# shahcompbio/MultiModalMuSig.jl

Hardware: AMD Instinct MI355X
Metric: E-step docs/sec (higher is better)
Workload: dtype f64; 1 GPU; LDA K=10 alpha=eta=0.1, 10000 docs x 96 SNV terms (BASELINE configs[1]), nnz(rank 0)=913480, one EM iteration per step; docs_rank0=10000, docs_total=10000, terms=96, topics=10, allreduce=none, comm_nranks=1, devices_visible=1

## Files before the change

include/mmmusig.h:

```cpp
#ifndef MMMUSIG_H
#define MMMUSIG_H

#include <stddef.h>
#include <stdint.h>

#ifdef __cplusplus
extern "C" {
#endif

#define MMM_VERSION 123

enum {
    MMM_OK = 0,
    MMM_DEFERRED = 1,
    MMM_ERR_ARG = -1,
    MMM_ERR_HIP = -2,
    MMM_ERR_RCCL = -3,
    MMM_ERR_UNSUPPORTED = -4,
    MMM_ERR_NUMERIC = -5,
    MMM_ERR_NO_DEVICE = -6
};

typedef struct mmm_ctx mmm_ctx;
typedef struct mmm_lda mmm_lda;
typedef struct mmm_ctm mmm_ctm;

int mmm_version(void);
int mmm_ctx_create(int device_id, mmm_ctx** out);
int mmm_ctx_destroy(mmm_ctx* ctx);
const char* mmm_last_error(const mmm_ctx* ctx);
int mmm_ctx_synchronize(mmm_ctx* ctx);
void* mmm_ctx_stream(mmm_ctx* ctx);
int mmm_ctx_device_name(mmm_ctx* ctx, char* buf, size_t n);

enum { MMM_BUILD_AUTO = 0,
       MMM_BUILD_SPARSE = 1,
       MMM_BUILD_DENSE = 2,
       MMM_BUILD_WIDE = 3 };
enum {
    MMM_OFF_LDA_PADDED_ROWS = 1 << 0,
    MMM_OFF_LDA_COUNT_ROWS = 1 << 1,
    MMM_OFF_LDA_ROWS16 = 1 << 2,
    MMM_OFF_LDA_LL_JOIN = 1 << 3,
    MMM_OFF_LDA_MERGED = 1 << 4,
    MMM_OFF_P2P_FOLDED = 1 << 5,
    MMM_OFF_CTM_PACKED = 1 << 6,
    MMM_OFF_CTM_CPL = 1 << 7,
    MMM_OFF_CTM_KFIT = 1 << 8,
    MMM_OFF_CTM_FUSED_GAUSS = 1 << 9,
    MMM_OFF_CTM_LL_ROWS = 1 << 10,
    MMM_OFF_LDA_EARLY_PROLOGUE = 1 << 11,
    MMM_OFF_CTM_PIPE_GAUSS = 1 << 12,
    MMM_OFF_CTM_SOLVE_ORDER = 1 << 13,
    MMM_OFF_ALL = (1 << 14) - 1
};
typedef struct {
    int lda_build;
    int ctm_build;
    int geometry_cus;
    int grid_blocks;
    int waves_per_block;
    int moment_blocks;
    int side_stream;
    int resident_cap;
    unsigned disable;
    int solve_lanes;
    int solve_waves;
    int reserved[5];
} mmm_tuning_opts;
void mmm_tuning_opts_default(mmm_tuning_opts* o);
int mmm_ctx_set_tuning(mmm_ctx* ctx, const mmm_tuning_opts* opts);
int mmm_ctx_get_tuning(const mmm_ctx* ctx, mmm_tuning_opts* out);
int mmm_ctx_profile_begin(mmm_ctx* ctx);
int mmm_ctx_profile_repeat(mmm_ctx* ctx, int repeat);
int mmm_ctx_profile_select(mmm_ctx* ctx, int phase);
int mmm_ctx_profile_end_phases(mmm_ctx* ctx, int n_spans[8], double total_ms[8]);
int mmm_ctx_profile_end(mmm_ctx* ctx, int* n_launches, double* total_ms);

#define MMM_UNIQUE_ID_BYTES 128
int mmm_comm_unique_id(char out[MMM_UNIQUE_ID_BYTES]);
int mmm_comm_init_rank(mmm_ctx* ctx, int nranks, int rank, const char id[MMM_UNIQUE_ID_BYTES]);
int mmm_comm_nranks(const mmm_ctx* ctx);
#define MMM_P2P_HANDLE_BYTES 64
const char* mmm_comm_transport(const mmm_ctx* ctx);
int mmm_p2p_local_handle(mmm_ctx* ctx, int nranks, char out[MMM_P2P_HANDLE_BYTES]);
int mmm_p2p_attach(mmm_ctx* ctx, int nranks, int rank, const char* handles);
int mmm_p2p_selftest(mmm_ctx* ctx, int* ok);
// ... 2 lines not shown
enum {
    MMM_LDA_LAMBDA = 0,
    MMM_LDA_ELNBETA = 1,
    MMM_LDA_BETA = 2,
    MMM_LDA_GAMMA = 3,
    MMM_LDA_ELNTHETA = 4,
    MMM_LDA_THETA = 5,
    MMM_LDA_PHI = 6,
    MMM_ILDA_LAMBDA = 7, MMM_ILDA_ELNBETA = 8, MMM_ILDA_BETA = 9
};
int mmm_lda_create(mmm_ctx* ctx, int D, int V, int K, double alpha, double eta, const int64_t* doc_ptr,
                   const int32_t* term, const int32_t* count, const double* lambda0, mmm_lda** out);
int mmm_ilda_create(mmm_ctx* ctx, int D, int V, int K, double alpha, int I, const int* J, const double* eta,
                    const int32_t* features, const int64_t* doc_ptr, const int32_t* term, const int32_t* count,
                    const double* lambda0, mmm_lda** out);
int mmm_lda_destroy(mmm_lda* m);
int mmm_lda_get(mmm_lda* m, int field, double* host, size_t n);
int mmm_lda_set(mmm_lda* m, int field, const double* host, size_t n);
int mmm_lda_set_hyper(mmm_lda* m, double alpha, const double* eta, int n_eta);
int mmm_lda_update_gamma(mmm_lda* m);
int mmm_lda_update_phi(mmm_lda* m);
int mmm_lda_update_lambda(mmm_lda* m);
int mmm_lda_update_beta(mmm_lda* m);
int mmm_lda_update_Elntheta(mmm_lda* m);
int mmm_lda_update_Elnbeta(mmm_lda* m);
int mmm_lda_update_theta(mmm_lda* m);
int mmm_lda_loglik(mmm_lda* m, double* ll);
int mmm_lda_elbo(mmm_lda* m, double* elbo, double terms[7]);
int mmm_lda_iterate(mmm_lda* m, int n_iter);
int mmm_lda_ll_history(mmm_lda* m, double* ll, int max_n, int* n);
int mmm_lda_geometry(const mmm_lda* m, int out[8]);
int mmm_lda_row_bytes(const mmm_lda* m);
int mmm_lda_prologue_moved(const mmm_lda* m);
int mmm_lda_fit(mmm_lda* m, int maxiter, double tol, double* ll_hist, int* n_iter, int* converged,
                double* elbo);
int mmm_lda_infer(mmm_lda* m, int unsmoothed, int maxiter, double tol, double* ll_hist, int* n_iter,
                  int* converged);

int mmm_lda_create_batch(mmm_ctx* ctx, int R, int D, int V, int K, double alpha, double eta, const int64_t* doc_ptr,
                         const int32_t* term, const int32_t* count, const double* lambda0, mmm_lda** out);
int mmm_lda_replicas(const mmm_lda* m);
int mmm_lda_select(mmm_lda* m, int r);
int mmm_lda_fit_batch(mmm_lda* m, int maxiter, double tol, double* ll_hist, int* n_iter, int* converged, double* elbo);

typedef struct {
    double xtol_rel;
    double xtol_abs;
    double nu_lower;
    int xtol_rule;
    int max_eval;
} mmm_solver_opts;
void mmm_solver_opts_default(mmm_solver_opts* o);

enum {
    MMM_CTM_MU = 0, MMM_CTM_SIGMA = 1, MMM_CTM_INVSIGMA = 2, MMM_CTM_GAMMA = 3, MMM_CTM_ELNPHI = 4,
    MMM_CTM_PHI = 5, MMM_CTM_LAMBDA = 6, MMM_CTM_NU = 7, MMM_CTM_ZETA = 8, MMM_CTM_PROPS = 9,
    MMM_CTM_THETA = 10, MMM_CTM_ALPHA = 11
};
int mmm_ctm_create(mmm_ctx* ctx, int D, int M, const int* K, const int* V, const double* alpha,
                   const int64_t* doc_ptr, const int32_t* term, const int32_t* count, const int* n_feat,
                   const int* J, const int32_t* features, const double* gamma0, const mmm_solver_opts* opts,
                   mmm_ctm** out);
int mmm_ctm_destroy(mmm_ctm* m);
int mmm_ctm_get(mmm_ctm* m, int field, double* host, size_t n);
int mmm_ctm_set(mmm_ctm* m, int field, const double* host, size_t n);
int mmm_ctm_update_zeta(mmm_ctm* m);
// ... 76 lines not shown
```

multimodalmusig.jl_amd/_lib.py:

```python
import ctypes as C
import os
import subprocess

import numpy as np

_HERE = os.path.dirname(os.path.abspath(__file__))
LIB_PATH = os.environ.get("MMM_LIB_PATH") or os.path.join(_HERE, "lib", "libmmmusig_hip.so")
_LIB = None

f64p = np.ctypeslib.ndpointer(dtype=np.float64, flags="C_CONTIGUOUS")
i64p = np.ctypeslib.ndpointer(dtype=np.int64, flags="C_CONTIGUOUS")
i32p = np.ctypeslib.ndpointer(dtype=np.int32, flags="C_CONTIGUOUS")
vp = C.c_void_p


class MmmError(RuntimeError):
    pass


class SolverOpts(C.Structure):
    _fields_ = [("xtol_rel", C.c_double), ("xtol_abs", C.c_double), ("nu_lower", C.c_double),
                ("xtol_rule", C.c_int), ("max_eval", C.c_int)]


# ... 15 lines not shown
    "mmm_ctx_stream": (vp, [vp]),
    "mmm_ctx_device_name": (C.c_int, [vp, C.c_char_p, C.c_size_t]),
    "mmm_ctx_profile_begin": (C.c_int, [vp]),
    "mmm_ctx_profile_repeat": (C.c_int, [vp, C.c_int]),
    "mmm_ctx_profile_select": (C.c_int, [vp, C.c_int]),
    "mmm_ctx_profile_end_phases": (C.c_int, [vp, C.POINTER(C.c_int), C.POINTER(C.c_double)]),
    "mmm_ctx_profile_end": (C.c_int, [vp, C.POINTER(C.c_int), C.POINTER(C.c_double)]),
    "mmm_comm_unique_id": (C.c_int, [C.c_char_p]),
    "mmm_comm_init_rank": (C.c_int, [vp, C.c_int, C.c_int, C.c_char_p]),
    "mmm_comm_transport": (C.c_char_p, [vp]),
    "mmm_p2p_local_handle": (C.c_int, [vp, C.c_int, C.c_char_p]),
    "mmm_p2p_attach": (C.c_int, [vp, C.c_int, C.c_int, C.c_char_p]),
    "mmm_p2p_selftest": (C.c_int, [vp, C.POINTER(C.c_int)]),
    "mmm_p2p_enable": (C.c_int, [vp, C.c_int]),
    "mmm_comm_nranks": (C.c_int, [vp]),
    "mmm_lda_create": (C.c_int, [vp, C.c_int, C.c_int, C.c_int, C.c_double, C.c_double, i64p, vp, vp, f64p, C.POINTER(vp)]),
    "mmm_ilda_create": (C.c_int, [vp, C.c_int, C.c_int, C.c_int, C.c_double, C.c_int, i32p, f64p, i32p, i64p, vp, vp, f64p, C.POINTER(vp)]),
    "mmm_lda_destroy": (C.c_int, [vp]),
    "mmm_lda_get": (C.c_int, [vp, C.c_int, f64p, C.c_size_t]),
    "mmm_lda_set": (C.c_int, [vp, C.c_int, f64p, C.c_size_t]),
    "mmm_lda_set_hyper": (C.c_int, [vp, C.c_double, f64p, C.c_int]),
    "mmm_lda_update_gamma": (C.c_int, [vp]),
    "mmm_lda_update_phi": (C.c_int, [vp]),
    "mmm_lda_update_lambda": (C.c_int, [vp]),
    "mmm_lda_update_beta": (C.c_int, [vp]),
    "mmm_lda_update_theta": (C.c_int, [vp]),
    "mmm_lda_loglik": (C.c_int, [vp, C.POINTER(C.c_double)]),
    "mmm_lda_elbo": (C.c_int, [vp, C.POINTER(C.c_double), vp]),
    "mmm_lda_iterate": (C.c_int, [vp, C.c_int]),
    "mmm_lda_ll_history": (C.c_int, [vp, vp, C.c_int, C.POINTER(C.c_int)]),
    "mmm_lda_geometry": (C.c_int, [vp, C.POINTER(C.c_int)]),
    "mmm_lda_row_bytes": (C.c_int, [vp]),
    "mmm_lda_prologue_moved": (C.c_int, [vp]),
    "mmm_lda_fit": (C.c_int, [vp, C.c_int, C.c_double, vp, C.POINTER(C.c_int), C.POINTER(C.c_int), C.POINTER(C.c_double)]),
    "mmm_solver_opts_default": (None, [C.POINTER(SolverOpts)]),
    "mmm_lda_infer": (C.c_int, [vp, C.c_int, C.c_int, C.c_double, vp, C.POINTER(C.c_int), C.POINTER(C.c_int)]),
    "mmm_ctm_create": (C.c_int, [vp, C.c_int, C.c_int, i32p, i32p, f64p, i64p, vp, vp, vp, vp, vp, f64p, C.POINTER(SolverOpts), C.POINTER(vp)]),
    "mmm_ctm_destroy": (C.c_int, [vp]),
    "mmm_ctm_get": (C.c_int, [vp, C.c_int, f64p, C.c_size_t]),
    "mmm_ctm_set": (C.c_int, [vp, C.c_int, f64p, C.c_size_t]),
    "mmm_ctm_update_zeta": (C.c_int, [vp]),
    "mmm_ctm_update_theta": (C.c_int, [vp]),
    "mmm_ctm_update_nu": (C.c_int, [vp]),
    "mmm_ctm_update_lambda": (C.c_int, [vp]),
    "mmm_ctm_update_mu": (C.c_int, [vp]),
    "mmm_ctm_update_Sigma": (C.c_int, [vp]),
    "mmm_ctm_update_gamma": (C.c_int, [vp]),
    "mmm_ctm_update_Elnphi": (C.c_int, [vp]),
    "mmm_ctm_update_props": (C.c_int, [vp]),
    "mmm_ctm_update_alpha": (C.c_int, [vp]),
    "mmm_ctm_update_phi": (C.c_int, [vp]),
    "mmm_ctm_loglik": (C.c_int, [vp, f64p]),
    "mmm_ctm_elbo": (C.c_int, [vp, C.POINTER(C.c_double), vp]),
    "mmm_ctm_objectives": (C.c_int, [vp, C.c_int, C.POINTER(C.c_double), f64p, C.POINTER(C.c_double), f64p]),
    "mmm_ctm_geometry": (C.c_int, [vp, C.POINTER(C.c_int)]),
    "mmm_debug_math": (C.c_int, [vp, C.c_int, C.c_size_t, f64p, vp, f64p]),
    "mmm_ctm_solver_stats": (C.c_int, [vp, C.POINTER(C.c_int64), C.POINTER(C.c_int64), C.POINTER(C.c_int64), vp, vp]),
    "mmm_ctm_events": (C.c_int, [vp, C.POINTER(C.c_int64)]),
    "mmm_lda_events": (C.c_int, [vp, C.POINTER(C.c_int64)]),
    "mmm_ctm_iterate": (C.c_int, [vp, C.c_int, C.c_int]),
    "mmm_ctm_ll_history": (C.c_int, [vp, vp, C.c_int, C.POINTER(C.c_int)]),
    "mmm_ctm_fit": (C.c_int, [vp, C.c_int, C.c_double, C.c_int, vp, C.POINTER(C.c_int), C.POINTER(C.c_int), C.POINTER(C.c_double)]),
    "mmm_ctm_infer": (C.c_int, [vp, C.c_int, C.c_int, C.c_double, vp, C.POINTER(C.c_int), C.POINTER(C.c_int)]),
    "mmm_ctm_create_batch": (C.c_int, [vp, C.c_int, C.c_int, C.c_int, i32p, i32p, f64p, i64p, vp, vp, vp, vp, vp, f64p, C.POINTER(SolverOpts), C.POINTER(vp)]),
    "mmm_ctm_replicas": (C.c_int, [vp]),
    "mmm_ctm_select": (C.c_int, [vp, C.c_int]),
# ... 35 lines not shown

def lib():
    global _LIB
    if _LIB is not None:
        return _LIB
    if not os.path.exists(LIB_PATH):
        raise MmmError("libmmmusig_hip.so is not built (%s missing): run `python -c 'import __graft_entry__ as g; g.build()'` "
                       "or `make -C multimodalmusig.jl_amd/csrc`. There is no CPU fallback." % LIB_PATH)
    L = C.CDLL(LIB_PATH, mode=C.RTLD_GLOBAL)
    for name, (res, args) in _SIGS.items():
        fn = getattr(L, name)
        fn.restype = res
        fn.argtypes = args
    _LIB = L
    return L


def check(rc, ctx_handle=None, what=""):
    if rc != 0:
        msg = lib().mmm_last_error(ctx_handle)
        raise MmmError("%s failed with status %d: %s" % (what or "libmmmusig_hip call", rc, (msg or b"").decode(errors="replace")))


_ALL_CTX = []


class TuningOpts(C.Structure):
    _fields_ = [("lda_build", C.c_int), ("ctm_build", C.c_int), ("geometry_cus", C.c_int), ("grid_blocks", C.c_int), ("waves_per_block", C.c_int),
                ("moment_blocks", C.c_int), ("side_stream", C.c_int), ("resident_cap", C.c_int), ("disable", C.c_uint), ("solve_lanes", C.c_int), ("solve_waves", C.c_int), ("reserved", C.c_int * 5)]


BUILDS = {"auto": 0, "sparse": 1, "dense": 2, "wide": 3}
OFF = {"lda_padded_rows": 1 << 0, "lda_count_rows": 1 << 1, "lda_rows16": 1 << 2, "lda_ll_join": 1 << 3, "lda_merged": 1 << 4, "p2p_folded": 1 << 5,
       "ctm_packed": 1 << 6, "ctm_cpl": 1 << 7, "ctm_kfit": 1 << 8, "ctm_fused_gauss": 1 << 9, "ctm_ll_rows": 1 << 10, "lda_early_prologue": 1 << 11, "ctm_pipe_gauss": 1 << 12, "ctm_solve_order": 1 << 13}


class Context:

    def __init__(self, device=0):
        self.h = vp()
        rc = lib().mmm_ctx_create(int(device), C.byref(self.h))
        if rc != 0:
            msg = lib().mmm_last_error(None)
            raise MmmError("mmm_ctx_create(device=%d) failed with status %d: %s -- the HIP path is the only path; "
                           "no CPU fallback exists" % (device, rc, (msg or b"").decode(errors="replace")))
        self.device = int(device)
        self.nranks, self.rank = 1, 0
        _ALL_CTX.append(self)

    def synchronize(self):
        check(lib().mmm_ctx_synchronize(self.h), self.h, "mmm_ctx_synchronize")

    def set_tuning(self, lda_build="auto", ctm_build="auto", geometry_cus=0, grid_blocks=0, waves_per_block=0, moment_blocks=0, side_stream=0,
                   resident_cap=0, disable=(), solve_lanes=0, solve_waves=0):
        t = TuningOpts()
        t.lda_build, t.ctm_build = BUILDS[lda_build], BUILDS[ctm_build]
        t.geometry_cus, t.grid_blocks, t.waves_per_block, t.moment_blocks = int(geometry_cus), int(grid_blocks), int(waves_per_block), int(moment_blocks)
        t.side_stream, t.resident_cap = int(side_stream), int(resident_cap)
        t.solve_lanes, t.solve_waves = int(solve_lanes), int(solve_waves)
        d = 0
        for name in ([disable] if isinstance(disable, str) else disable):
            d |= OFF[name]
        t.disable = d
        check(lib().mmm_ctx_set_tuning(self.h, C.byref(t)), self.h, "mmm_ctx_set_tuning")
        return self

    def get_tuning(self):
# ... 111 lines not shown
```

multimodalmusig.jl_amd/csrc/lda.hip:

```cpp
#include <memory>
#include "dev_math.h"
#include "mmm_logtab.h"
#include "mmm_exptab.h"
#include "mmm_internal.h"

namespace {

constexpr int kWavesPerBlock = 4;
constexpr int kBlock = kWavesPerBlock * MMM_WAVE;
constexpr int kMaxWavesE = 12;

struct LdaDev {
    int D, V, K;
    const int64_t* doc_ptr;
    const int2* tc;
    double alpha, eta;
    const int2* ell;
    const int* dense;
    int Vp;
    const unsigned short* dense16;
};

__device__ __forceinline__ int row_slot(int w, int slp) { return (w & 15) * slp + (w >> 4); }
__device__ __forceinline__ int row16_count(unsigned w0, unsigned w1, unsigned w2, unsigned w3, int c)
// ... 152 lines not shown
    DevBuf<double> lambda[3], Elnbeta[3], expElnbeta[3], beta[3], gamma[3], Elntheta[3];
    DevBuf<double> theta, phi;
    DevBuf<double> partial, stats[2], scratch, llpart, llpart2, elbopart, ll_hist;
    int n_ll = 0;
    DevBuf<LdaCtl> ctl;
    int t = 0, n_hist = 0, cap_hist = 0;
    bool inflight = false;
    bool phi_valid = false;
    bool phi_from_prev = false;
    bool gnext_valid = false;
    bool ll_pending = false;
    bool theta_valid = false;
    bool attr_e[2] = {false, false}, attr_m = false, attr_mm[3] = {false, false, false};
    int cap_mm[3] = {-1, -1, -1}, cap_m = -1;
    DevBuf<unsigned long long> cells;
    DevBuf<unsigned long long> fcells;
    unsigned int kseq = 0;
    bool stop_seen = false;
    bool lag_ll = true;
    bool phi_table_beta = false;
    bool single_step = false;
    bool wide = false;
    DevBuf<int64_t> term_ptr;
    DevBuf<int2> tpost;
    DevBuf<double> aexp;
    DevBuf<double> aexp_next;
    int aexp_for = -1;
    bool pro_used = false;
    DevBuf<double> tabT;
    int stats_waves = 1;
    bool attr_big = false, attr_bigs = false;
    int grid_e = 1, waves_e = 8, grid_s = 1;
    size_t lds_e = 0, lds_tab = 0;
    bool ilda = false;
    IldaDesc ids{};
    DevBuf<int> features;
    DevBuf<double> ilam[3], iEln[3], ibeta[3];
    int R = 1, sel = 0;
    std::vector<int> rep_t, rep_hist;
    PinnedCtl pin;
    LdaDev dev() const { return LdaDev{D, V, K, doc_ptr.p, tc.p, alpha, eta, tc_ell.p, (drows && !cnt16.p) ? cnt_dense.p : nullptr, 16 * SLs, cnt16.p}; }
    int cur() const { return t % 3; }
    Ring ring(DevBuf<double>* b) const { return Ring{{b[0].p, b[1].p, b[2].p}}; }
    double* tab(DevBuf<double>* b, int s) const { return b[s].p + (size_t)sel * V * K; }
    double* doc(DevBuf<double>* b, int s) const { return b[s].p + (size_t)sel * K * D; }
    LdaCtl* ctlp() const { return ctl.p + sel; }
    double* hist() const { return ll_hist.p + (size_t)sel * cap_hist; }
};

namespace {

int pick_kp(int K)
{
    static const int opts[] = {2, 4, 6, 8, 10, 12, 16, 20, 24, 32};
    for (int o : opts) if (K <= o) return o;
    if (K <= 64 * kLdaSlots) return (K + 1) & ~1;
    return -1;
}

#define MMM_KP_SWITCH(m, ...)                                                                                   \
    switch ((m)->KP) {                                                                                          \
        case 2: { constexpr int KPV = 2; __VA_ARGS__ } break;                                                          \
        case 4: { constexpr int KPV = 4; __VA_ARGS__ } break;                                                          \
        case 6: { constexpr int KPV = 6; __VA_ARGS__ } break;                                                          \
        case 8: { constexpr int KPV = 8; __VA_ARGS__ } break;                                                          \
        case 10: { constexpr int KPV = 10; __VA_ARGS__ } break;                                                        \
// ... 3 lines not shown
        case 24: { constexpr int KPV = 24; __VA_ARGS__ } break;                                                        \
        case 32: { constexpr int KPV = 32; __VA_ARGS__ } break;                                                        \
        default: return mmm_fail((m)->ctx, MMM_ERR_UNSUPPORTED, "LDA: K=%d has no build on this path (the LDS builds stop at 32 topics)", (m)->K);    \
    }

template <typename Kern>
int set_lds(mmm_ctx* ctx, Kern kern, size_t lds)
{
    if (lds > 48 * 1024) MMM_HIP(ctx, hipFuncSetAttribute((const void*)kern, hipFuncAttributeMaxDynamicSharedMemorySize, (int)lds));
    return MMM_OK;
}

template <class Kern>
int residency_cap(mmm_lda* m, Kern kern, size_t lds, int* cap)
{
    mmm_ctx* ctx = m->ctx;
    int nb = 0;
    MMM_HIP(ctx, hipOccupancyMaxActiveBlocksPerMultiprocessor(&nb, (const void*)kern, 1024, lds));
    *cap = nb * std::max(1, ctx->num_cu - 4);
    if (m->tune.resident_cap > 0) *cap = std::min(*cap, m->tune.resident_cap);
    return MMM_OK;
}

template <int KPV, int LV, bool LLV, int VT, bool SG, bool RB>
int go_estep3(mmm_lda* m, const EstepArgs& a)
{
    mmm_ctx* ctx = m->ctx;
    auto k = k_lda_estep<KPV, LV, LLV, VT, SG, RB>;
    if (!m->attr_e[LLV]) { int rc = set_lds(ctx, k, m->lds_e); if (rc) return rc; m->attr_e[LLV] = true; }
    hipLaunchKernelGGL(k, dim3(m->grid_e, RB ? m->R : 1), dim3(m->waves_e * MMM_WAVE), m->lds_e, ctx->stream, a);
    return MMM_OK;
}

template <int KPV, int LV, bool LLV, int VT, bool RB>
int go_estep2(mmm_lda* m, const EstepArgs& a)
{
    if constexpr (LV == 16 && KPV <= 12) { if (m->single_step) return go_estep3<KPV, LV, LLV, VT, true, RB>(m, a); }
    return go_estep3<KPV, LV, LLV, VT, false, RB>(m, a);
}

template <int KPV, int LV, bool LLV, bool RB = false>
int go_estep(mmm_lda* m, const EstepArgs& a)
{
    if constexpr (LV == 16 && (KPV == 8 || KPV == 10)) { if (m->V == 96) return go_estep2<KPV, LV, LLV, 96, RB>(m, a); }
    return go_estep2<KPV, LV, LLV, 0, RB>(m, a);
}

template <int KPV, int SLV, bool RB = false>
int go_dense(mmm_lda* m, const EstepArgs& a)
{
    if constexpr (KPV * SLV <= 64) {
        mmm_ctx* ctx = m->ctx;
        const bool c16 = m->cnt16.p != nullptr;
        auto k = c16 ? k_lda_estep_dense<KPV, SLV, true, RB> : k_lda_estep_dense<KPV, SLV, false, RB>;
        if (!m->attr_d) { int rc = set_lds(ctx, k, m->lds_d); if (rc) return rc; m->attr_d = true; }
        hipLaunchKernelGGL(k, dim3(m->grid_e, RB ? m->R : 1), dim3(m->waves_e * MMM_WAVE), m->lds_d, ctx->stream, a, (const int*)m->cnt_dense.p, (const unsigned short*)m->cnt16.p);
        return MMM_OK;
    } else return mmm_fail(m->ctx, MMM_ERR_UNSUPPORTED, "LDA: no dense-row build for KP=%d SL=%d", KPV, SLV);
}

int dense_slots(int V) { return V <= 32 ? 2 : (V <= 48 ? 3 : (V <= 96 ? 6 : (V <= 128 ? 8 : 0))); }

template <bool RB = false>
int launch_estep(mmm_lda* m, const EstepArgs& a)
{
    mmm_ctx* ctx = m->ctx;
    int rc = MMM_OK;
    if (m->dense && !a.do_ll) {
        MMM_KP_SWITCH(m, {
// ... 488 lines not shown

static int lda_create_impl(mmm_ctx* ctx, int D, int V, int K, double alpha, double eta, const int64_t* doc_ptr, const int32_t* term,
                           const int32_t* count, const double* lambda0, int I, const int* J, const double* eta_i, const int32_t* features,
                           mmm_lda** out, int R = 1)
{
    if (!ctx) return MMM_ERR_ARG;
    MMM_CHECK(ctx, out && doc_ptr && lambda0, "mmm_lda_create: NULL argument");
    const bool ilda = I > 0;
    int SJ = 0;
    if (ilda) {
        MMM_CHECK(ctx, J && eta_i && features, "mmm_ilda_create: NULL argument");
        if (I > kIldaMaxI) return mmm_fail(ctx, MMM_ERR_UNSUPPORTED, "mmm_ilda_create: I=%d features (max %d)", I, kIldaMaxI);
        for (int i = 0; i < I; ++i) { MMM_CHECK(ctx, J[i] >= 1, "mmm_ilda_create: J[%d] < 1", i); SJ += J[i]; }
        if (SJ > kIldaMaxSJ) return mmm_fail(ctx, MMM_ERR_UNSUPPORTED, "mmm_ilda_create: sum(J)=%d (max %d)", SJ, kIldaMaxSJ);
        for (int i = 0; i < I; ++i) for (int v = 0; v < V; ++v)
            MMM_CHECK(ctx, features[(size_t)i * V + v] >= 0 && features[(size_t)i * V + v] < J[i], "mmm_ilda_create: feature value out of range (i=%d v=%d)", i, v);
    }
    MMM_CHECK(ctx, D >= 0 && V >= 1 && K >= 1, "mmm_lda_create: bad sizes D=%d V=%d K=%d", D, V, K);
    *out = nullptr;
    const int KP = pick_kp(K);
    if (KP < 0) return mmm_fail(ctx, MMM_ERR_UNSUPPORTED, "mmm_lda_create: K=%d not supported (max 256: an LDS column block of 512 K bytes per wave)", K);
    const int64_t nnz = doc_ptr[D];
    MMM_CHECK(ctx, doc_ptr[0] == 0 && nnz >= 0 && (nnz == 0 || (term && count)), "mmm_lda_create: bad CSR");
    std::vector<int2> tc((size_t)nnz);
    for (int d = 0; d < D; ++d) MMM_CHECK(ctx, doc_ptr[d + 1] >= doc_ptr[d], "mmm_lda_create: doc_ptr not monotone at %d", d);
    for (int64_t e = 0; e < nnz; ++e) {
        MMM_CHECK(ctx, term[e] >= 0 && term[e] < V && count[e] >= 0, "mmm_lda_create: entry %lld out of range (term %d, count %d)", (long long)e, term[e], count[e]);
        tc[(size_t)e] = make_int2(term[e], count[e]);
    }
    const int L = (K <= 15) ? 16 : (K <= 31 ? 32 : 64);
    const int G = MMM_WAVE / L;
    const int ncu = mmm_geo_cus(ctx);
    const size_t tabB = (size_t)KP * V * sizeof(double);
    bool dense = false, drows = false;
    const int SL = dense_slots(V);
    {
        const int build = ctx->tune.lda_build;
        const int dmode = build == MMM_BUILD_DENSE ? 1 : (build == MMM_BUILD_AUTO ? -1 : 0);
        const bool drows_env = !mmm_off(ctx->tune, MMM_OFF_LDA_COUNT_ROWS);
        const bool rshape = SL > 0 && L == 16 && D > 0 && build != MMM_BUILD_WIDE;
        const bool shape = rshape && KP >= 4 && KP * SL <= 64;
        const bool dense_enough = 2 * nnz >= (int64_t)D * V;
        bool dup = false;
        if (rshape && ((shape && dmode != 0) || (drows_env && dense_enough))) {
            std::vector<int> seen((size_t)V, -1);
            for (int d = 0; d < D && !dup; ++d)
                for (int64_t e = doc_ptr[d]; e < doc_ptr[d + 1]; ++e) { if (seen[(size_t)term[e]] == d) { dup = true; break; } seen[(size_t)term[e]] = d; }
        }
        const bool big = D > 12 * G * ncu;
        const bool off32 = (int64_t)D * K * 8 < ((int64_t)1 << 32) && (int64_t)D * 16 * (SL + 1) * 4 < ((int64_t)1 << 32);
        dense = shape && !dup && off32 && dmode != 0 && (dmode > 0 || (big && dense_enough));
        drows = drows_env && rshape && !dup && dense_enough;
    }
    const bool small = !dense && (V <= 96) && KP <= 12 && ((D + 12 * G - 1) / (12 * G) <= ncu) && ctx->tune.grid_blocks == 0;
    const int swaves = ctx->tune.waves_per_block > 0 ? std::min(12, ctx->tune.waves_per_block) : std::max(kMinWavesSingle, std::min(12, (D + G * ncu - 1) / (G * ncu)));
    int waves = small ? swaves : 8;
    auto lds_for = [&](int w) { return tabB * (2 + w) + (size_t)2 * w * G * KP * sizeof(double); };
    while (waves > 1 && lds_for(waves) > (small ? 150 : 80) * 1024) --waves;
    const bool wide = lds_for(waves) > 160 * 1024 || KP > 32 || (ctx->tune.lda_build == MMM_BUILD_WIDE) || (ctx->tune.lda_build == MMM_BUILD_AUTO && KP >= 32);
    if (R > 1 && wide) {
        const char* why = ctx->tune.lda_build == MMM_BUILD_WIDE ? "lda_build = MMM_BUILD_WIDE takes the wide path (tables through L2)"
                        : KP > 32 ? "K > 32 topics take the wide path (no LDS build)"
                        : ctx->tune.lda_build == MMM_BUILD_AUTO && KP >= 32 ? "K >= 25 topics take the wide path under MMM_BUILD_AUTO"
                        : "the K x V tables and one slab exceed LDS (wide path)";
        return mmm_fail(ctx, MMM_ERR_UNSUPPORTED, "mmm_lda_create_batch: K=%d V=%d: %s, which has no batched build -- fit such shapes on single handles", K, V, why);
    }

    MMM_HIP(ctx, hipSetDevice(ctx->device));
    std::unique_ptr<mmm_lda> guard(new mmm_lda());
    mmm_lda* m = guard.get();
    m->tune = ctx->tune;
    m->ctx = ctx; m->D = D; m->V = V; m->K = K; m->KP = KP; m->L = L; m->nnz = nnz; m->alpha = alpha; m->eta = eta;
    m->R = R; m->rep_t.assign((size_t)R, 0); m->rep_hist.assign((size_t)R, 0);
    m->waves_e = waves; m->lds_e = wide ? 0 : lds_for(waves); m->lds_tab = tabB; m->wide = wide;
    m->dense = dense && !wide; m->SL = SL; m->drows = (dense || drows) && !wide;
    if (!wide && ctx->tune.waves_per_block > 0) { const int w = ctx->tune.waves_per_block; if (w >= 1 && w <= (small ? kMaxWavesE : 8) && lds_for(w) <= 160 * 1024) { m->waves_e = w; m->lds_e = lds_for(w); } }
    const size_t VK = (size_t)V * K, KD = (size_t)K * D, Rs = (size_t)R;
    const int docs_per_block = m->waves_e * G;
    const int blocks_per_cu = wide ? 8 : std::max(1, std::min<int>((small ? 12 : 8) / m->waves_e, (int)((160 * 1024) / m->lds_e)));
    m->single_step = !wide && small && (int64_t)m->waves_e * G * ncu * blocks_per_cu >= D;
    m->grid_e = std::max(1, std::min((D + docs_per_block - 1) / docs_per_block, ncu * blocks_per_cu));
    if (wide) m->grid_e = std::max(1, std::min((D + kWavesPerBlock - 1) / kWavesPerBlock, ncu * blocks_per_cu));
    if (ctx->tune.grid_blocks > 0) m->grid_e = ctx->tune.grid_blocks;
    if ((int64_t)m->grid_e * docs_per_block < D) m->single_step = false;
    if (m->dense)
        m->lds_d = sizeof(double) * ((size_t)16 * SL * KP + (size_t)m->waves_e * 16 * SL * KP + (size_t)m->waves_e * G * KP + (size_t)m->waves_e * MMM_WAVE * KP);
    if (m->dense && m->lds_d > 160 * 1024) { m->dense = false; m->drows = drows && !wide; }
    m->grid_s = std::max(1, std::min((D + kWavesPerBlock - 1) / kWavesPerBlock, ncu * 4));
    const int grid_max = std::max(m->grid_e, m->grid_s);
#define A(buf, n) do { hipError_t e_ = m->buf.alloc(n); if (e_ != hipSuccess) { int rc = mmm_fail(ctx, MMM_ERR_HIP, "hipMalloc(" #buf "): %s", hipGetErrorString(e_)); return rc; } } while (0)
    A(doc_ptr, (size_t)D + 1); A(tc, (size_t)nnz);
    for (int i = 0; i < 3; ++i) { A(lambda[i], Rs * VK); A(Elnbeta[i], Rs * VK); A(expElnbeta[i], Rs * VK); A(beta[i], Rs * VK); A(gamma[i], Rs * KD); A(Elntheta[i], Rs * KD); }
    A(theta, KD); A(phi, (size_t)K * nnz);
    const size_t VKp = (size_t)((V + 15) & ~15) * K;
    A(partial, wide ? 1 : Rs * m->grid_e * VKp); A(stats[0], Rs * (VKp + 16)); A(stats[1], Rs * (VKp + 16)); A(scratch, VK + 16); A(llpart, Rs * grid_max);
    A(llpart2, Rs * 1024); A(elbopart, (size_t)m->grid_s * 5 + 8 * Rs);
    A(ctl, Rs); A(cells, 2 * 1024);
    if (m->single_step && !ilda) A(aexp_next, KD);
    if (ilda) {
        A(fcells, (size_t)2 * 512 * 16);
        A(features, (size_t)I * V);
        for (int i = 0; i < 3; ++i) { A(ilam[i], (size_t)SJ * K); A(iEln[i], (size_t)SJ * K); A(ibeta[i], (size_t)SJ * K); }
    }
#undef A
    hipStream_t st = ctx->stream;
    MMM_HIP(ctx, hipMemcpyAsync(m->doc_ptr.p, doc_ptr, sizeof(int64_t) * (D + 1), hipMemcpyHostToDevice, st));
    if (nnz) MMM_HIP(ctx, hipMemcpyAsync(m->tc.p, tc.data(), sizeof(int2) * nnz, hipMemcpyHostToDevice, st));
    std::vector<int64_t> tptr;
    std::vector<int2> tpost;
    if (wide) {
        tptr.assign((size_t)V + 1, 0);
        for (int64_t e = 0; e < nnz; ++e) tptr[(size_t)term[e] + 1]++;
        for (int v = 0; v < V; ++v) tptr[(size_t)v + 1] += tptr[(size_t)v];
        tpost.resize((size_t)nnz);
        std::vector<int64_t> fill(tptr.begin(), tptr.end() - 1);
        for (int d = 0; d < D; ++d)
            for (int64_t e = doc_ptr[d]; e < doc_ptr[d + 1]; ++e) tpost[(size_t)fill[(size_t)term[e]]++] = make_int2(d, count[e]);
// ... 313 lines not shown
{
    if (!m) return MMM_ERR_ARG;
    MMM_NOT_ON_BATCH(m, "mmm_lda_iterate");
    mmm_ctx* ctx = m->ctx;
    if (int rc = mmm_ctx_usable(ctx, "mmm_lda_iterate")) return rc;
    MMM_HIP(ctx, hipSetDevice(ctx->device));
    MMM_CHECK(ctx, n_iter >= 0, "mmm_lda_iterate: n_iter < 0");
    m->aexp_for = -1;
    if (m->stop_seen) {
        hipLaunchKernelGGL(k_ctl_clear_stop, dim3(1), dim3(1), 0, ctx->stream, m->ctl.p);
        MMM_LAUNCH_CHECK(ctx);
        m->stop_seen = false;
    }
    return fused_passes(m, n_iter, -1.0, 0);
}

int mmm_lda_geometry(const mmm_lda* m, int out[8])
{
    if (!m || !out) return MMM_ERR_ARG;
    out[0] = m->L; out[1] = m->grid_e; out[2] = m->waves_e; out[3] = m->single_step ? 1 : 0; out[4] = m->wide ? 1 : 0;
    out[5] = m->dense ? 1 : 0; out[6] = m->dense ? m->SL : 0; out[7] = m->KP;
    return MMM_OK;
}

int mmm_lda_row_bytes(const mmm_lda* m)
{
    if (!m || m->wide) return 0;
    if (m->drows) return (m->cnt16.p ? 2 : 4) * 16 * m->SLs;
    if (m->tc_ell.p && !m->dense) return 8 * m->V;
    return 0;
}

int mmm_lda_prologue_moved(const mmm_lda* m) { return (m && m->pro_used) ? 1 : 0; }

int mmm_lda_ll_history(mmm_lda* m, double* ll, int max_n, int* n)
{
    if (!m || !n) return MMM_ERR_ARG;
    mmm_ctx* ctx = m->ctx;
    int rc = prepare_call(m);
    if (rc || (rc = flush_ll(m, nullptr))) return rc;
    const int cnt = std::min(max_n, m->n_hist);
    if (cnt > 0 && ll) MMM_HIP(ctx, hipMemcpyAsync(ll, m->hist() + (m->n_hist - cnt), sizeof(double) * cnt, hipMemcpyDeviceToHost, ctx->stream));
    MMM_HIP(ctx, hipStreamSynchronize(ctx->stream));
    if ((rc = mmm_p2p_check(ctx))) return rc;
    *n = cnt;
    return MMM_OK;
}

int mmm_lda_events(mmm_lda* m, int64_t out[4])
{
    if (!m || !out) return MMM_ERR_ARG;
    mmm_ctx* ctx = m->ctx;
    int rc = prepare_call(m);
    if (rc || (rc = flush_ll(m, nullptr))) return rc;
    std::vector<double> ll((size_t)std::max(m->n_hist, 0));
    if (!ll.empty()) MMM_HIP(ctx, hipMemcpyAsync(ll.data(), m->hist(), sizeof(double) * ll.size(), hipMemcpyDeviceToHost, ctx->stream));
    MMM_HIP(ctx, hipStreamSynchronize(ctx->stream));
    if ((rc = mmm_p2p_check(ctx))) return rc;
    out[0] = out[1] = out[2] = out[3] = 0;
    for (double v : ll) if (!std::isfinite(v)) ++out[2];
    return MMM_OK;
}

static int lda_elbo_enqueue(mmm_lda* m, double* acc)
{
    mmm_ctx* ctx = m->ctx;
// ... 265 lines not shown
```

multimodalmusig.jl_amd/csrc/lda_estep.cuh:

```cuda
__device__ __forceinline__ void lds_wave_sync()
{
    __builtin_amdgcn_fence(__ATOMIC_SEQ_CST, "wavefront");
    __builtin_amdgcn_wave_barrier();
}

template <int KP, bool LL>
__device__ __forceinline__ void lda_chunk(const int2 tcv, const bool act, const int V, const double (&av)[KP], double (&acc)[KP],
                                          const double* __restrict__ sB, const double* __restrict__ sBeta,
                                          const double* __restrict__ myT, double* __restrict__ slab, double& ll_acc)
{
    const double n = (double)tcv.y;
    if (LL) {
        const double* bc = sBeta + tcv.x;
        double p0 = 0.0, p1 = 0.0;
#pragma unroll
        for (int k = 0; k + 1 < KP; k += 2) { p0 = fma(myT[k], bc[k * V], p0); p1 = fma(myT[k + 1], bc[(k + 1) * V], p1); }
        if (KP & 1) p0 = fma(myT[KP - 1], bc[(KP - 1) * V], p0);
        ll_acc = fma(n, dev_log_pos(p0 + p1), ll_acc);
        __builtin_amdgcn_sched_barrier(0);
    }
    const double* bcol = sB + tcv.x;
    if (KP >= 20) {
        double s0 = 0.0, s1 = 0.0;
#pragma unroll
// ... 133 lines not shown
            const int2* __restrict__ row = a.c.ell + (size_t)(valid ? d : 0) * V;
#pragma unroll
            for (int j = 0; j < PRE; ++j) {
                int c = j + rot; if (c >= NCHR) c -= NCHR;
                const int w = c * L + l;
                tcp[j] = (valid && j < NCHR && w < V) ? row[w] : make_int2(-1, 0);
            }
        } else if (!rows && (SINGLE || first)) {
#pragma unroll
            for (int j = 0; j < PRE; ++j) {
                int c = j + rot; if (c >= nch) c -= nch;
                const int w = c * L + l;
                tcp[j] = ((j < nch) && (w < W)) ? tcd[w] : make_int2(-1, 0);
            }
        }
        double el = 0.0;
        if (ext) { if (l < KP) myA[l] = gk; }
        else {
            const double S = group_sum<L>(gk);
            const double ps = dev_digamma_pos(l < K ? gk : S);
            const double psS = __shfl(ps, g * L + K, MMM_WAVE);
            el = ps - psS;
            if (l < KP) myA[l] = (l < K) ? ar_exp(el) : 0.0;
        }
        if (LL) {
            const double Sp = group_sum<L>(gp);
            if (l < KP) myT[l] = (l < K) ? gp / Sp : 0.0;
        }
        if (first) {
            if (stop) return;
            if (SINGLE) {
#pragma unroll
                for (int q = 0; q < TB; ++q) { const int i = tid + q * (int)blockDim.x; if (i < KP * V) sB[i] = tb[q]; }
            }
            __syncthreads();
            first = false;
            MMM_STAMP(2);
        } else lds_wave_sync();
        if (!ext && valid && l < K) Eln[(size_t)d * K + l] = el;
        MMM_STAMP(3);
        int2 tcn[PRE];
        double gkn = 0.0, gpn = 0.0;
        int d2 = 0; bool valid2 = false; int64_t start2 = 0; int W2 = 0;
        const bool more = !SINGLE && base + stride < D;
        if (more) {
            const int nch1 = rows ? NCHR : (W1 + L - 1) / L;
            const int rot1 = nch1 > 0 ? g % nch1 : 0;
            const int2* __restrict__ tcd1 = a.c.tc + start1;
            if (drows) {
                const int* __restrict__ row = a.c.dense + (size_t)(valid1 ? d1 : 0) * a.c.Vp;
                const unsigned short* __restrict__ row16 = a.c.dense16 + (size_t)(valid1 ? d1 : 0) * a.c.Vp;
                const bool h16 = a.c.dense16 != nullptr;
                const int slp = a.c.Vp >> 4;
                if (L == 16 && h16) {
                    const unsigned* __restrict__ r32 = (const unsigned*)(row16 + (size_t)l * slp);
                    const unsigned w0 = r32[0], w1 = r32[1], w2 = r32[2], w3 = r32[3];
#pragma unroll
                    for (int j = 0; j < PRE; ++j) {
                        int c = j + rot1; if (c >= NCHR) c -= NCHR;
                        const int w = c * L + l;
                        const bool in = valid1 && j < NCHR && w < V;
                        const int n = in ? row16_count(w0, w1, w2, w3, c) : 0;
                        tcn[j] = make_int2(n > 0 ? w : -1, n);
                    }
                } else
#pragma unroll
// ... 69 lines not shown
#pragma unroll
        for (int j = 0; j < PRE; ++j) tcp[j] = tcn[j];
        d1 = d2; valid1 = valid2; start1 = start2; W1 = W2;
        lds_wave_sync();
    }
    MMM_STAMP(6);
    if (LL) ll_acc = wave_sum(ll_acc);
    __syncthreads();
    if (LL && lane == 0) sA[wid] = ll_acc;
    double* out = a.partial + (size_t)blockIdx.x * K * a.pstride;
    if constexpr (RB) out += (size_t)blockIdx.y * gridDim.x * K * a.pstride;
    for (int i = tid; i < K * V; i += blockDim.x) {
        double v8[kMaxWavesE];
#pragma unroll
        for (int w = 0; w < kMaxWavesE; ++w) v8[w] = (w < NW) ? sSlab[(size_t)w * KP * V + i] : 0.0;
        double s = 0.0;
#pragma unroll
        for (int w = 0; w < kMaxWavesE; ++w) s += v8[w];
        out[a.pstride == V ? i : (i / V) * a.pstride + i % V] = s;
    }
    if (LL) {
        __syncthreads();
        if (tid == 0) {
            double s = 0.0;
            for (int w = 0; w < NW; ++w) s += sA[w];
            if constexpr (RB) a.llpart[(size_t)blockIdx.y * gridDim.x + blockIdx.x] = s;
            else a.llpart[blockIdx.x] = s;
        }
    }
    MMM_STAMP(7);
}


template <class T> __device__ __forceinline__ T* at_byte(T* base, unsigned off) { return (T*)((char*)base + off); }
typedef unsigned short mmm_us2 __attribute__((ext_vector_type(2)));

template <int KP, int SL, bool C16, bool RB = false>
__global__ __launch_bounds__(512, 2) void k_lda_estep_dense(EstepArgs a, const int* __restrict__ cnt, const unsigned short* __restrict__ cnt16)
{
    extern __shared__ __attribute__((aligned(16))) double smem[];
    constexpr int L = 16, G = MMM_WAVE / L, Vp = L * SL;
    MMM_STAMP(0);
    const int t = a.t;
    const int stop = rep<RB>(a.ctl, 1)->stop;
    const double* __restrict__ gam = a.gamma.s[t % 3];
    double* __restrict__ gnext = a.gamma.s[(t + 1) % 3];
    double* __restrict__ Eln = a.Elntheta.s[t % 3];
    const double* __restrict__ eB = a.expElnbeta.s[(t + 2) % 3];
    if constexpr (RB) {
        const size_t KD = (size_t)a.c.K * a.c.D, VK = (size_t)a.c.V * a.c.K;
        gam = rep<RB>(gam, KD); gnext = rep<RB>(gnext, KD); Eln = rep<RB>(Eln, KD); eB = rep<RB>(eB, VK);
    }
    const int K = a.c.K, D = a.c.D, V = a.c.V;
    const int NW = blockDim.x >> 6;
    const int tid = threadIdx.x, lane = tid & 63, wid = tid >> 6;
    const int g = lane / L, l = lane % L;
    double* sT = smem;
    double* sSlab = sT + (size_t)Vp * KP;
    double* sA = sSlab + (size_t)NW * Vp * KP;
    double* sR = sA + (size_t)NW * G * KP;
    double* slab = sSlab + (size_t)wid * Vp * KP;
    double* myA = sA + ((size_t)wid * G + g) * KP;
    double* myR = sR + (size_t)wid * MMM_WAVE * KP;
    const int stride = gridDim.x * NW * G;
    int base = (blockIdx.x * NW + wid) * G;
    __shared__ __attribute__((aligned(16))) double sTabs[MMM_EXPTAB_N + MMM_LOGTAB_N];
// ... 132 lines not shown
```

multimodalmusig.jl_amd/models.py:

```python
import ctypes as C

import numpy as np

from . import _lib
from ._lib import MmmError, check, lib
from .utils import doc_totals, pack_lda, pack_mm

_F = {"lambda": 0, "Elnbeta": 1, "beta": 2, "gamma": 3, "Elntheta": 4, "theta": 5, "phi": 6, "ilambda": 7, "iElnbeta": 8, "ibeta": 9}


class _PerDocView:

    def __init__(self, getter, setter, D):
        self._get, self._set, self._D = getter, setter, D

    def __len__(self):
        return self._D

    def __getitem__(self, d):
        return self._get(d)

    def __setitem__(self, d, value):
        self._set(d, value)

# ... 96 lines not shown
    def ϕ(self):
        def get(d):
            flat = self._get("phi")
            a, b = int(self._doc_ptr[d]), int(self._doc_ptr[d + 1])
            return flat[self.K * a:self.K * b].reshape(b - a, self.K).T.copy()

        def put(d, value):
            flat = self._get("phi")
            a, b = int(self._doc_ptr[d]), int(self._doc_ptr[d + 1])
            value = np.asarray(value, dtype=np.float64)
            if value.shape != (self.K, b - a):
                raise ValueError("ϕ[d] must be K x W_d")
            flat[self.K * a:self.K * b] = value.T.ravel()
            self._set("phi", flat)
        return _PerDocView(get, put, self.D)

    @ϕ.setter
    def ϕ(self, docs):
        flat = np.concatenate([np.asarray(p, dtype=np.float64).T.ravel() for p in docs]) if len(docs) else np.zeros(0)
        self._set("phi", flat)

    def phi_flat(self):
        return self._get("phi").reshape(-1, self.K)

    def events(self):
        out = (C.c_int64 * 4)()
        check(lib().mmm_lda_events(self._h, out), self.ctx.h, "events")
        return {"n_capped": int(out[0]), "n_nonfinite": int(out[1]), "n_nonfinite_ll": int(out[2])}

    def geometry(self):
        g = (C.c_int * 8)()
        check(lib().mmm_lda_geometry(self._h, g), self.ctx.h, "geometry")
        return {"L": g[0], "grid_e": g[1], "waves_e": g[2], "single_step": g[3], "wide": g[4], "dense": g[5], "SL": g[6], "KP": g[7],
                "row_bytes": int(lib().mmm_lda_row_bytes(self._h)), "prologue_moved": int(lib().mmm_lda_prologue_moved(self._h))}

    def close(self):
        if self._h:
            lib().mmm_lda_destroy(self._h)
            self._h = C.c_void_p()

    def __del__(self):
        try:
            self.close()
        except Exception:
            pass


class _FactorList:

    def __init__(self, model, name):
        self._m, self._name = model, name

    def __len__(self):
        return self._m.I

    def __getitem__(self, i):
        m = self._m
        flat = m._get(self._name)
        return flat[m._ioff[i]:m._ioff[i + 1]].reshape(m.J[i], m.K, order="F").copy()

    def __setitem__(self, i, value):
        m = self._m
        flat = m._get(self._name)
        value = np.asarray(value, dtype=np.float64)
        if value.shape != (m.J[i], m.K):
            raise ValueError("%s[%d] must be J_i x K" % (self._name, i))
        flat[m._ioff[i]:m._ioff[i + 1]] = value.ravel(order="F")
# ... 159 lines not shown
```

Baseline: 559.1 million docs/s.

## Add block-level sufficient-statistics E-step kernel storing per-doc ratios in LDS

```diff
diff --git a/include/mmmusig.h b/include/mmmusig.h
--- a/include/mmmusig.h
+++ b/include/mmmusig.h
@@ -52,7 +52,8 @@
     MMM_OFF_LDA_EARLY_PROLOGUE = 1 << 11,
     MMM_OFF_CTM_PIPE_GAUSS = 1 << 12,
     MMM_OFF_CTM_SOLVE_ORDER = 1 << 13,
-    MMM_OFF_ALL = (1 << 14) - 1
+    MMM_OFF_LDA_BLOCK_STATS = 1 << 14,
+    MMM_OFF_ALL = (1 << 15) - 1
 };
 typedef struct {
     int lda_build;
@@ -121,6 +122,7 @@
 int mmm_lda_geometry(const mmm_lda* m, int out[8]);
 int mmm_lda_row_bytes(const mmm_lda* m);
 int mmm_lda_prologue_moved(const mmm_lda* m);
+int mmm_lda_stats_build(const mmm_lda* m);
 int mmm_lda_fit(mmm_lda* m, int maxiter, double tol, double* ll_hist, int* n_iter, int* converged,
                 double* elbo);
 int mmm_lda_infer(mmm_lda* m, int unsmoothed, int maxiter, double tol, double* ll_hist, int* n_iter,
diff --git a/multimodalmusig.jl_amd/_lib.py b/multimodalmusig.jl_amd/_lib.py
--- a/multimodalmusig.jl_amd/_lib.py
+++ b/multimodalmusig.jl_amd/_lib.py
@@ -71,6 +71,7 @@
     "mmm_lda_geometry": (C.c_int, [vp, C.POINTER(C.c_int)]),
     "mmm_lda_row_bytes": (C.c_int, [vp]),
     "mmm_lda_prologue_moved": (C.c_int, [vp]),
+    "mmm_lda_stats_build": (C.c_int, [vp]),
     "mmm_lda_fit": (C.c_int, [vp, C.c_int, C.c_double, vp, C.POINTER(C.c_int), C.POINTER(C.c_int), C.POINTER(C.c_double)]),
     "mmm_solver_opts_default": (None, [C.POINTER(SolverOpts)]),
     "mmm_lda_infer": (C.c_int, [vp, C.c_int, C.c_int, C.c_double, vp, C.POINTER(C.c_int), C.POINTER(C.c_int)]),
@@ -172,7 +173,7 @@
 
 BUILDS = {"auto": 0, "sparse": 1, "dense": 2, "wide": 3}
 OFF = {"lda_padded_rows": 1 << 0, "lda_count_rows": 1 << 1, "lda_rows16": 1 << 2, "lda_ll_join": 1 << 3, "lda_merged": 1 << 4, "p2p_folded": 1 << 5,
-       "ctm_packed": 1 << 6, "ctm_cpl": 1 << 7, "ctm_kfit": 1 << 8, "ctm_fused_gauss": 1 << 9, "ctm_ll_rows": 1 << 10, "lda_early_prologue": 1 << 11, "ctm_pipe_gauss": 1 << 12, "ctm_solve_order": 1 << 13}
+       "ctm_packed": 1 << 6, "ctm_cpl": 1 << 7, "ctm_kfit": 1 << 8, "ctm_fused_gauss": 1 << 9, "ctm_ll_rows": 1 << 10, "lda_early_prologue": 1 << 11, "ctm_pipe_gauss": 1 << 12, "ctm_solve_order": 1 << 13, "lda_block_stats": 1 << 14}
 
 
 class Context:
diff --git a/multimodalmusig.jl_amd/csrc/lda.hip b/multimodalmusig.jl_amd/csrc/lda.hip
--- a/multimodalmusig.jl_amd/csrc/lda.hip
+++ b/multimodalmusig.jl_amd/csrc/lda.hip
@@ -208,6 +208,8 @@
     bool attr_big = false, attr_bigs = false;
     int grid_e = 1, waves_e = 8, grid_s = 1;
     size_t lds_e = 0, lds_tab = 0;
+    bool block_stats = false;
+    size_t lds_b = 0; bool attr_b = false;
     bool ilda = false;
     IldaDesc ids{};
     DevBuf<int> features;
@@ -277,9 +279,20 @@
     return MMM_OK;
 }
 
+template <int KPV, int VT, bool RB>
+int go_estep_block(mmm_lda* m, const EstepArgs& a)
+{
+    mmm_ctx* ctx = m->ctx;
+    auto k = k_lda_estep_block<KPV, VT, RB>;
+    if (!m->attr_b) { int rc = set_lds(ctx, k, m->lds_b); if (rc) return rc; m->attr_b = true; }
+    hipLaunchKernelGGL(k, dim3(m->grid_e, RB ? m->R : 1), dim3(m->waves_e * MMM_WAVE), m->lds_b, ctx->stream, a);
+    return MMM_OK;
+}
+
 template <int KPV, int LV, bool LLV, int VT, bool RB>
 int go_estep2(mmm_lda* m, const EstepArgs& a)
 {
+    if constexpr (LV == 16 && KPV <= 12 && !LLV) { if (m->single_step && m->block_stats) return go_estep_block<KPV, VT, RB>(m, a); }
     if constexpr (LV == 16 && KPV <= 12) { if (m->single_step) return go_estep3<KPV, LV, LLV, VT, true, RB>(m, a); }
     return go_estep3<KPV, LV, LLV, VT, false, RB>(m, a);
 }
@@ -834,7 +847,7 @@
     const int G = MMM_WAVE / L;
     const int ncu = mmm_geo_cus(ctx);
     const size_t tabB = (size_t)KP * V * sizeof(double);
-    bool dense = false, drows = false;
+    bool dense = false, drows = false, dup_terms = false;
     const int SL = dense_slots(V);
     {
         const int build = ctx->tune.lda_build;
@@ -844,7 +857,8 @@
         const bool shape = rshape && KP >= 4 && KP * SL <= 64;
         const bool dense_enough = 2 * nnz >= (int64_t)D * V;
         bool dup = false;
-        if (rshape && ((shape && dmode != 0) || (drows_env && dense_enough))) {
+        const bool block_shape = L == 16 && KP <= 12 && V <= 96;
+        if ((rshape && ((shape && dmode != 0) || (drows_env && dense_enough))) || block_shape) {
             std::vector<int> seen((size_t)V, -1);
             for (int d = 0; d < D && !dup; ++d)
                 for (int64_t e = doc_ptr[d]; e < doc_ptr[d + 1]; ++e) { if (seen[(size_t)term[e]] == d) { dup = true; break; } seen[(size_t)term[e]] = d; }
@@ -853,6 +867,7 @@
         const bool off32 = (int64_t)D * K * 8 < ((int64_t)1 << 32) && (int64_t)D * 16 * (SL + 1) * 4 < ((int64_t)1 << 32);
         dense = shape && !dup && off32 && dmode != 0 && (dmode > 0 || (big && dense_enough));
         drows = drows_env && rshape && !dup && dense_enough;
+        dup_terms = dup;
     }
     const bool small = !dense && (V <= 96) && KP <= 12 && ((D + 12 * G - 1) / (12 * G) <= ncu) && ctx->tune.grid_blocks == 0;
     const int swaves = ctx->tune.waves_per_block > 0 ? std::min(12, ctx->tune.waves_per_block) : std::max(kMinWavesSingle, std::min(12, (D + G * ncu - 1) / (G * ncu)));
@@ -885,6 +900,8 @@
     if (wide) m->grid_e = std::max(1, std::min((D + kWavesPerBlock - 1) / kWavesPerBlock, ncu * blocks_per_cu));
     if (ctx->tune.grid_blocks > 0) m->grid_e = ctx->tune.grid_blocks;
     if ((int64_t)m->grid_e * docs_per_block < D) m->single_step = false;
+    m->block_stats = m->single_step && L == 16 && KP <= 12 && !dup_terms && !mmm_off(ctx->tune, MMM_OFF_LDA_BLOCK_STATS);
+    m->lds_b = sizeof(double) * ((size_t)KP * V + (size_t)m->waves_e * G * (((size_t)V + 15) & ~(size_t)15) + (size_t)m->waves_e * G * KP);
     if (m->dense)
         m->lds_d = sizeof(double) * ((size_t)16 * SL * KP + (size_t)m->waves_e * 16 * SL * KP + (size_t)m->waves_e * G * KP + (size_t)m->waves_e * MMM_WAVE * KP);
     if (m->dense && m->lds_d > 160 * 1024) { m->dense = false; m->drows = drows && !wide; }
@@ -1264,6 +1281,8 @@
 }
 
 int mmm_lda_prologue_moved(const mmm_lda* m) { return (m && m->pro_used) ? 1 : 0; }
+
+int mmm_lda_stats_build(const mmm_lda* m) { return (m && m->block_stats) ? 1 : 0; }
 
 int mmm_lda_ll_history(mmm_lda* m, double* ll, int max_n, int* n)
 {
diff --git a/multimodalmusig.jl_amd/csrc/lda_estep.cuh b/multimodalmusig.jl_amd/csrc/lda_estep.cuh
--- a/multimodalmusig.jl_amd/csrc/lda_estep.cuh
+++ b/multimodalmusig.jl_amd/csrc/lda_estep.cuh
@@ -189,6 +189,7 @@
             if (SINGLE) {
 #pragma unroll
                 for (int q = 0; q < TB; ++q) { const int i = tid + q * (int)blockDim.x; if (i < KP * V) sB[i] = tb[q]; }
+                for (int i = tid + TB * (int)blockDim.x; i < KP * V; i += blockDim.x) sB[i] = (i < K * V) ? eB[i] : 0.0;
             }
             __syncthreads();
             first = false;
@@ -324,6 +325,166 @@
 }
 
 
+template <int KP>
+__device__ __forceinline__ double lda_chunk_r(const int v, const double n, const bool act, const int V, const double (&av)[KP], double (&acc)[KP],
+                                              const double* __restrict__ sB)
+{
+    const double* bcol = sB + v;
+    double b[KP], s0 = 0.0, s1 = 0.0;
+#pragma unroll
+    for (int k = 0; k < KP; ++k) b[k] = bcol[k * V];
+#pragma unroll
+    for (int k = 0; k + 1 < KP; k += 2) { s0 = fma(av[k], b[k], s0); s1 = fma(av[k + 1], b[k + 1], s1); }
+    if (KP & 1) s0 = fma(av[KP - 1], b[KP - 1], s0);
+    const double r = act ? n * dev_rcp(s0 + s1) : 0.0;
+#pragma unroll
+    for (int k = 0; k < KP; ++k) acc[k] = fma(b[k], r, acc[k]);
+    return r;
+}
+
+template <int KP, int VT, bool RB = false>
+__global__ __launch_bounds__(kMaxWavesE * MMM_WAVE, 3) void k_lda_estep_block(EstepArgs a)
+{
+    static_assert(KP <= 12 && KP % 2 == 0, "topic pairs, table of <= 5 registers per thread");
+    extern __shared__ __attribute__((aligned(16))) double smem[];
+    constexpr int L = 16, G = MMM_WAVE / L, PRE = 96 / L;
+    MMM_STAMP(0);
+    const int t = a.t;
+    const int stop = rep<RB>(a.ctl, 1)->stop;
+    const double* __restrict__ gam = a.gamma.s[t % 3];
+    double* __restrict__ gnext = a.gamma.s[(t + 1) % 3];
+    double* __restrict__ Eln = a.Elntheta.s[t % 3];
+    const double* __restrict__ eB = a.expElnbeta.s[(t + 2) % 3];
+    if constexpr (RB) {
+        const size_t KD = (size_t)a.c.K * a.c.D, VK = (size_t)a.c.V * a.c.K;
+        gam = rep<RB>(gam, KD); gnext = rep<RB>(gnext, KD); Eln = rep<RB>(Eln, KD); eB = rep<RB>(eB, VK);
+    }
+    const int K = a.c.K, D = a.c.D;
+    const int V = VT ? VT : a.c.V;
+    const int NCHR = VT ? (VT + L - 1) / L : (V + L - 1) / L;
+    const int Vs = NCHR * L;
+    const int NW = blockDim.x >> 6, ND = NW * G;
+    const int tid = threadIdx.x, lane = tid & 63, wid = tid >> 6;
+    const int g = lane / L, l = lane % L;
+    double* sB = smem;
+    double* sR = sB + (size_t)KP * V;
+    double* sA = sR + (size_t)ND * Vs;
+    double* myR = sR + (size_t)(wid * G + g) * Vs;
+    double* myA = sA + (size_t)(wid * G + g) * KP;
+
+    const int d = (blockIdx.x * NW + wid) * G + g;
+    const bool valid = d < D;
+    const bool ext = !RB && a.aexp != nullptr;
+    const double gk = ext ? ((valid && l < K) ? a.aexp[(size_t)d * K + l] : 0.0) : ((valid && l < K) ? gam[(size_t)d * K + l] : (l < K ? 1.0 : 0.0));
+    const bool drows = a.c.dense != nullptr || a.c.dense16 != nullptr;
+    const bool rows = drows || a.c.ell != nullptr;
+    const int64_t start = (valid && !rows) ? a.c.doc_ptr[d] : 0;
+    const int W = (valid && !rows) ? (int)(a.c.doc_ptr[d + 1] - start) : 0;
+    constexpr int TB = KP <= 10 ? 4 : 5;
+    double tb[TB];
+#pragma unroll
+    for (int q = 0; q < TB; ++q) { const int i = tid + q * (int)blockDim.x; tb[q] = (i < K * V) ? eB[i] : 0.0; }
+    if (!drows) for (int i = tid; i < ND * Vs; i += blockDim.x) sR[i] = 0.0;
+    MMM_STAMP(1);
+
+    int tv[PRE]; double tn[PRE];
+    const int nch = rows ? NCHR : (W + L - 1) / L;
+    if (drows) {
+        const int* __restrict__ row = a.c.dense + (size_t)(valid ? d : 0) * a.c.Vp;
+        const unsigned short* __restrict__ row16 = a.c.dense16 + (size_t)(valid ? d : 0) * a.c.Vp;
+        const bool h16 = a.c.dense16 != nullptr;
+        const int slp = a.c.Vp >> 4;
+        if (h16) {
+            const unsigned* __restrict__ r32 = (const unsigned*)(row16 + (size_t)l * slp);
+            const unsigned w0 = r32[0], w1 = r32[1], w2 = r32[2], w3 = r32[3];
+#pragma unroll
+            for (int j = 0; j < PRE; ++j) {
+                const int w = j * L + l;
+                const int n = (valid && j < NCHR && w < V) ? row16_count(w0, w1, w2, w3, j) : 0;
+                tv[j] = n > 0 ? w : -1; tn[j] = (double)n;
+            }
+        } else
+#pragma unroll
+        for (int j = 0; j < PRE; ++j) {
+            const int w = j * L + l;
+            const int n = (valid && j < NCHR && w < V) ? row[row_slot(w, slp)] : 0;
+            tv[j] = n > 0 ? w : -1; tn[j] = (double)n;
+        }
+    } else {
+        const int2* __restrict__ src = rows ? a.c.ell + (size_t)(valid ? d : 0) * V : a.c.tc + start;
+        const int lim = rows ? (valid ? V : 0) : W;
+#pragma unroll
+        for (int j = 0; j < PRE; ++j) {
+            const int w = j * L + l;
+            const int2 p = (j < nch && w < lim) ? src[w] : make_int2(-1, 0);
+            tv[j] = p.x; tn[j] = (double)p.y;
+        }
+    }
+    double el = 0.0, al = gk;
+    if (!ext) {
+        const double S = group_sum<L>(gk);
+        const double ps = dev_digamma_pos(l < K ? gk : S);
+        const double psS = __shfl(ps, g * L + K, MMM_WAVE);
+        el = ps - psS;
+        al = (l < K) ? ar_exp(el) : 0.0;
+    }
+    if (l < KP) myA[l] = al;
+    if (stop) return;
+#pragma unroll
+    for (int q = 0; q < TB; ++q) { const int i = tid + q * (int)blockDim.x; if (i < KP * V) sB[i] = tb[q]; }
+    for (int i = tid + TB * (int)blockDim.x; i < KP * V; i += blockDim.x) sB[i] = (i < K * V) ? eB[i] : 0.0;
+    __syncthreads();
+    MMM_STAMP(2);
+    if (!ext && valid && l < K) Eln[(size_t)d * K + l] = el;
+    MMM_STAMP(3);
+    double av[KP], acc[KP];
+#pragma unroll
+    for (int k = 0; k < KP; ++k) { av[k] = myA[k]; acc[k] = 0.0; }
+    int nchmax = nch;
+    if (!rows) {
+        nchmax = max(nchmax, __shfl_xor(nchmax, 32, MMM_WAVE));
+        nchmax = max(nchmax, __shfl_xor(nchmax, 16, MMM_WAVE));
+        nchmax = __builtin_amdgcn_readfirstlane(nchmax);
+    }
+#pragma unroll
+    for (int j = 0; j < PRE; ++j) {
+        if (j < nchmax) {
+            const bool act = tv[j] >= 0;
+            const double r = lda_chunk_r<KP>(act ? tv[j] : 0, tn[j], act, V, av, acc, sB);
+            if (drows) myR[j * L + l] = r;
+            else if (act) myR[tv[j]] = r;
+        }
+    }
+    MMM_STAMP(4);
+    double mine = 0.0;
+#pragma unroll
+    for (int k = 0; k < KP; ++k) { const double tot = group_sum<L>(acc[k]); if (l == k) mine = tot; }
+    if (valid && l < K) gnext[(size_t)d * K + l] = fma(al, mine, a.c.alpha);
+    MMM_STAMP(5);
+    __syncthreads();
+    MMM_STAMP(6);
+    double* out = a.partial + (size_t)blockIdx.x * K * a.pstride;
+    if constexpr (RB) out += (size_t)blockIdx.y * gridDim.x * K * a.pstride;
+    for (int i = tid; i < (KP / 2) * V; i += blockDim.x) {
+        const int kp = VT ? i / VT : i / V, v = i - kp * V, k = 2 * kp;
+        const double* rc = sR + v;
+        const double* ac = sA + k;
+        double t0 = 0.0, t1 = 0.0;
+#pragma unroll 2
+        for (int dd = 0; dd < ND; dd += G) {
+            double rr[G], a0[G], a1[G];
+#pragma unroll
+            for (int q = 0; q < G; ++q) { rr[q] = rc[(size_t)(dd + q) * Vs]; a0[q] = ac[(dd + q) * KP]; a1[q] = ac[(dd + q) * KP + 1]; }
+#pragma unroll
+            for (int q = 0; q < G; ++q) { t0 = fma(a0[q], rr[q], t0); t1 = fma(a1[q], rr[q], t1); }
+        }
+        if (k < K) out[k * a.pstride + v] = sB[k * V + v] * t0;
+        if (k + 1 < K) out[(k + 1) * a.pstride + v] = sB[(k + 1) * V + v] * t1;
+    }
+    MMM_STAMP(7);
+}
+
+
 template <class T> __device__ __forceinline__ T* at_byte(T* base, unsigned off) { return (T*)((char*)base + off); }
 typedef unsigned short mmm_us2 __attribute__((ext_vector_type(2)));
 
diff --git a/multimodalmusig.jl_amd/models.py b/multimodalmusig.jl_amd/models.py
--- a/multimodalmusig.jl_amd/models.py
+++ b/multimodalmusig.jl_amd/models.py
@@ -152,7 +152,8 @@
         g = (C.c_int * 8)()
         check(lib().mmm_lda_geometry(self._h, g), self.ctx.h, "geometry")
         return {"L": g[0], "grid_e": g[1], "waves_e": g[2], "single_step": g[3], "wide": g[4], "dense": g[5], "SL": g[6], "KP": g[7],
-                "row_bytes": int(lib().mmm_lda_row_bytes(self._h)), "prologue_moved": int(lib().mmm_lda_prologue_moved(self._h))}
+                "row_bytes": int(lib().mmm_lda_row_bytes(self._h)), "prologue_moved": int(lib().mmm_lda_prologue_moved(self._h)),
+                "block_stats": int(lib().mmm_lda_stats_build(self._h))}
 
     def close(self):
         if self._h:
```

Result: faster. 623.6 million docs/s, median of 6 (+11.5%).
